# prime-slam/octreelib

Hardware: AMD Instinct MI355X
Metric: Mpoints/s insert+subdivide+RANSAC (higher is better)
Workload: dtype f64; 1 GPU; BASELINE config 3: Grid 1 m voxels, 10000000 planar points per GPU (scene 32x32x32 voxels), insert + subdivide(len>64) + map_leaf_points_cuda_ransac(H=1024, k=6, thr=0.01, poses_per_batch=10) incl. apply_mask; points_per_gpu=10000000, K=64, hypotheses=1024, leaves=575543

## Files before the change

octreelib_amd/csrc/ransac.hip:

```cpp
#include <algorithm>
#include <cstdlib>
#include <type_traits>

#include "forest.h"
#include "lookback.h"
#include "wave_utils.h"

namespace {

__device__ __forceinline__ double div_by_small_int(double c, int k) {
  const double kd = (double)k;
  const double zh = 1.0 / kd;
  const double zl = fma(-kd, zh, 1.0) / kd;
  const double a = fabs(c);
  if (!((int(a > 1e-290) | int(c == 0.0)) & int(a < 1e290))) return c / kd;
  return copysign(fma(c, zh, c * zl), c);
}

__device__ __forceinline__ bool coord_in_fast_range(double v) {
  const uint32_t hi = (uint32_t)__double2hiint(v), lo = (uint32_t)__double2loint(v);
  const uint32_t e = (hi >> 20) & 0x7FFu;
  return (e - (1023u - 30u)) <= 60u || (hi | lo) == 0u;
}

// ... 132 lines not shown
      if (i == 0) {
        xx = rx * rx;
        yy = ry * ry;
        zz = rz * rz;
      } else {
        xx += rx * rx;
        yy += ry * ry;
        zz += rz * rz;
      }
      xy += rx * ry;
      xz += rx * rz;
      yz += ry * rz;
    }
  }
  plane_from_moments(cx, cy, cz, xx, xy, xz, yy, yz, zz, plane, fast);
}

__device__ __forceinline__ double plane_distance(double a, double b, double c, double d, double x,
                                                 double y, double z) {
  return fabs(((a * x + b * y) + c * z) + d);
}

constexpr int rs_minwaves(int threads, int kt) { return threads == 64 && kt > 0 ? 5 : 4; }
constexpr int RS_BIG_PER_CU = 16;
constexpr int RS_BIG_THREADS = 256;
constexpr int RS_BIG_HPL = 1024 / RS_BIG_THREADS;
constexpr int RS_SMALL_THREADS = 128;
constexpr int RS_TINY_THREADS = 64;
constexpr int RS_PER_CU = 64, RS_SMALL_PER_CU = 128, RS_TINY_PER_CU = 256;
constexpr int RS_KMAX = 16;
constexpr int RS_STAGE1_SLACK = 2;
constexpr int RS_STAGE2_MIN = 6;
constexpr int RS_STAGE2_RING = 128;

struct __attribute__((aligned(32))) BlockDesc {
  uint32_t pstart;
  int32_t n;
  int64_t vstart;
  uint32_t pspill;
  uint32_t pad[3];
};

struct RansacOut {
  uint8_t* mask;
  float* plane;
  int32_t* count;
  int32_t* index;
};

__device__ __forceinline__ int sample_index_exact(double r, int n, int64_t vstart) {
  const double v = r * (double)n + (double)vstart;
  const int g = (int)((int64_t)(int)v - vstart);
  return g < n ? g : n;
}

__device__ __forceinline__ int sample_index_cached(double r, int n, bool* risky) {
  const double x = r * (double)n;
  const int g0 = (int)x;
  *risky = (x - (double)g0) > (1.0 - 0x1p-20);
  return g0 < n ? g0 : n;
}

__device__ __forceinline__ void plane_streamed(const double* __restrict__ hyp_row, int k, const BlockDesc& d,
                                               const double* __restrict__ xyz, float (&plane)[4]) {
  auto point = [&](int i) {
    const int g = sample_index_exact(hyp_row[i], d.n, d.vstart);
// ... 270 lines not shown
#ifdef RS_COUNTS
constexpr int RS_NSTAMPS = 24;
__device__ unsigned long long g_rs_stamps[RS_NSTAMPS];
#define RS_COUNT_INIT unsigned long long _rs_acc[RS_NSTAMPS] = {0, 0, 0, 0, 0, 0, 0, 0, 0, 0, 0, 0, 0, 0, 0, 0,  \
                                                                0, 0, 0, 0, 0, 0, 0, 0};                             \
                      const unsigned long long _rs_m0 = __builtin_amdgcn_s_memtime(),                      \
                                               _rs_r0 = __builtin_amdgcn_s_memrealtime()
#define RS_COUNT(k, v) _rs_acc[k] += (unsigned long long)(v)
#define RS_COUNT_FLUSH                                                                  \
  do {                                                                                  \
    if (threadIdx.x == 0) {                                                             \
      _rs_acc[0] = __builtin_amdgcn_s_memtime() - _rs_m0;                               \
      _rs_acc[1] = __builtin_amdgcn_s_memrealtime() - _rs_r0;                           \
      _rs_acc[10] += 1;                                                                 \
      for (int _k = 0; _k < RS_NSTAMPS; ++_k) atomicAdd(&g_rs_stamps[_k], _rs_acc[_k]); \
    }                                                                                   \
  } while (0)
#else
#define RS_COUNT_INIT do {} while (0)
#define RS_COUNT(k, v) do {} while (0)
#define RS_COUNT_FLUSH do {} while (0)
#endif

template <int THREADS, int HPL, int KT, bool FULLH, bool PT>
__global__ __launch_bounds__(THREADS, rs_minwaves(THREADS, KT)) void k_ransac(
    const double* __restrict__ xyz, const BlockDesc* __restrict__ sdesc,
    const uint32_t* __restrict__ lo_ptr, const uint32_t* __restrict__ hi_ptr, const double* __restrict__ hyp, int H,
    int k_rt, double thr, RansacOut out, const uint2* __restrict__ pos_tab, int no_prescreen) {
  static_assert(!PT || (KT > 0 && KT <= 6), "the position table packs up to six positions and their risk bits");
  static_assert(THREADS * HPL <= 1024, "hypothesis index in 10 bits");
  constexpr bool PRE = PT && KT >= 3 && HPL >= 2;
  constexpr int W = THREADS / 64;
  constexpr bool PARK = PRE && W == 1;
  constexpr int KS = KT > 0 ? KT : RS_KMAX;
  constexpr int GW = (KS + 3) / 4;
  constexpr int PRE_LIST = THREADS == 64 ? 512 : 256;
  constexpr bool OWN_LIST = PRE && W > 1;
  __shared__ uint16_t s_surv_all[OWN_LIST ? W : 1][OWN_LIST ? PRE_LIST : 1];
  uint16_t* const s_surv_own = s_surv_all[OWN_LIST ? (threadIdx.x >> 6) : 0];
  const int k = KT > 0 ? KT : k_rt;
  __shared__ double s_pts[3][3][THREADS];
  __shared__ uint32_t s_wbest[2][W];
  __shared__ float s_wplane[2][W][4];
  __shared__ f4 s_loc[3][THREADS];
  static_assert(!(PRE && W == 1) || PRE_LIST * sizeof(uint16_t) <= sizeof(s_loc[0]), "the survivor list fits an s_loc buffer");
  __shared__ float s_wext[3][W];
  __shared__ uint32_t s_wfast[3][W];
  const int lo = lo_ptr ? (int)*lo_ptr : 0;
  const int hi = (int)*hi_ptr;
  const int nbs = hi - lo;
  const int C = (nbs + (int)gridDim.x - 1) / (int)gridDim.x;
  int j = lo + (int)blockIdx.x * C;
  const int j_end = min(hi, j + C);
  if (j >= j_end) return;
  float ext_carry = 0.f;
  uint32_t fast_carry = 0;
  BlockDesc cur = sdesc[j];
  BlockDesc nxt = cur;
  if (j + 1 < j_end) nxt = sdesc[j + 1];
  {
    double px = 0.0, py = 0.0, pz = 0.0;
    if ((int)threadIdx.x <= cur.n) {
      const int64_t p = ((int)threadIdx.x < cur.n) ? (int64_t)cur.pstart + threadIdx.x : (int64_t)cur.pspill;
      px = xyz[3 * p];
      py = xyz[3 * p + 1];
      pz = xyz[3 * p + 2];
      s_pts[0][0][threadIdx.x] = px;
      s_pts[0][1][threadIdx.x] = py;
      s_pts[0][2][threadIdx.x] = pz;
    }
    stage_local<THREADS>(threadIdx.x, xyz[3 * (int64_t)cur.pstart], xyz[3 * (int64_t)cur.pstart + 1],
                         xyz[3 * (int64_t)cur.pstart + 2], cur, px, py, pz, s_loc[0], s_wext[0], s_wfast[0],
                         W == 1 ? &ext_carry : nullptr, W == 1 ? &fast_carry : nullptr);
  }
  __syncthreads();
  int buf = 0, par = 0;
  RS_COUNT_INIT;
  for (;;) {
    unsigned tx = threadIdx.x;
    asm volatile("" : "+v"(tx));
    const bool has_next = j + 1 < j_end;
    BlockDesc nxt2 = nxt;
    if (j + 2 < j_end) nxt2 = sdesc[j + 2];
    double rx = 0.0, ry = 0.0, rz = 0.0;
    auto pre_here = [&]() {
      unsigned t = tx;
      if constexpr (PARK) asm volatile("" : "+v"(t));
      return has_next && (int)t <= nxt.n;
    };
    const int nbuf = buf == 2 ? 0 : buf + 1;
    uint16_t* const s_surv = PARK ? (uint16_t*)&s_loc[nbuf][0] : s_surv_own;
    auto prefetch = [&]() {
      if (pre_here()) {
        const int64_t p = ((int)tx < nxt.n) ? (int64_t)nxt.pstart + tx : (int64_t)nxt.pspill;
        rx = xyz[3 * p];
        ry = xyz[3 * p + 1];
        rz = xyz[3 * p + 2];
      }
    };
    auto park = [&]() {
      if (pre_here()) {
        s_pts[nbuf][0][tx] = rx;
        s_pts[nbuf][1][tx] = ry;
        s_pts[nbuf][2][tx] = rz;
      }
    };
    double nox = 0.0, noy = 0.0, noz = 0.0;
    if constexpr (!PARK) {
      prefetch();
      if (has_next) {
        nox = xyz[3 * (int64_t)nxt.pstart];
        noy = xyz[3 * (int64_t)nxt.pstart + 1];
        noz = xyz[3 * (int64_t)nxt.pstart + 2];
      }
    }
    const int n = cur.n;
    const int be = (int)cur.pad[1];
    const double* __restrict__ lx = s_pts[buf][0];
    const double* __restrict__ ly = s_pts[buf][1];
    const double* __restrict__ lz = s_pts[buf][2];

    RS_COUNT(8, 1);
    RS_COUNT(11, n);
    float extent = W == 1 ? ext_carry : s_wext[buf][0];
#pragma unroll
    for (int w = 1; w < W; ++w) extent = fmaxf(extent, s_wext[buf][w]);
    uint32_t fastw = W == 1 ? fast_carry : s_wfast[buf][0];
#pragma unroll
    for (int w = 1; w < W; ++w) fastw &= s_wfast[buf][w];
    const bool blk_fast = __builtin_amdgcn_readfirstlane((int)fastw) != 0;
    const bool blk_sane = thr >= 0x1p-40 && thr <= 0x1p40 && extent < 0x1p60f;
    const bool fast_screen = blk_fast && thr >= 0x1p-40 && thr <= 0x1p40;
    const f4* __restrict__ loc = s_loc[buf];
    struct BlkConst {
      double ox, oy, oz;
      double delta_blk, dprime_thr, thr2;
      float nthr2;
      float delta_blk_f, thr2_f, dprime_thr_f;
    };
    auto blk_consts = [&]() {
      double th = thr;
      if constexpr (PARK) asm volatile("" : "+s"(th));
      BlkConst c;
      c.ox = lx[0]; c.oy = ly[0]; c.oz = lz[0];
      c.delta_blk = fma(0x1p-23 * 9.0, (double)extent,
                        0x1p-49 * (fabs(c.ox) + fabs(c.oy) + fabs(c.oz) + (double)extent + 1.0));
      c.dprime_thr = 0x1p-21 * (th * th);
      c.thr2 = th + th;
      c.nthr2 = -(float)(th * th);
      c.delta_blk_f = (float)c.delta_blk * 0x1.0002p0f;
      c.thr2_f = (float)(th + th) * 0x1.0002p0f;
      c.dprime_thr_f = (float)c.dprime_thr * 0x1.0002p0f;
      return c;
    };
    const BlkConst bc0 = blk_consts();
    auto consts_here = [&]() {
      if constexpr (PARK) return blk_consts();
      else return bc0;
    };
    const double ox = bc0.ox, oy = bc0.oy, oz = bc0.oz;

    uint32_t gpk[GW], rk = 0;
    float fa = 0.f, fb = 0.f, fc = 0.f, fd = 0.f, sto = 0.f, sdl = 0.f;
    int cnt = 0;
    auto load_pos = [&](const int t, const bool act) {
#pragma unroll
      for (int w = 0; w < GW; ++w) gpk[w] = 0;
      rk = 0;
      if constexpr (PT) {
        const uint2 e = pos_tab[(size_t)n * (size_t)H + (size_t)(act ? t : 0)];
        gpk[0] = e.x;
        if (GW > 1) gpk[GW - 1] = e.y & 0xFFFFu;
        rk = e.y >> 16;
      } else if (act) {
        const double* __restrict__ row = hyp + (int64_t)t * k;
#pragma unroll
        for (int i = 0; i < KS; ++i) {
          if (i < k) {
            bool risky;
            const int g = sample_index_cached(row[i], n, &risky);
            gpk[i >> 2] |= (uint32_t)g << (8 * (i & 3));
            rk |= (risky || g == n) ? (1u << i) : 0u;
          }
        }
      }
    };
    auto fit = [&](const int t, const bool act) {
      cnt = 0;
      fa = fb = fc = fd = sto = sdl = 0.f;
      if (FULLH || act) {
        const BlkConst bc = consts_here();
        const double ox = bc.ox, oy = bc.oy, oz = bc.oz, delta_blk = bc.delta_blk, dprime_thr = bc.dprime_thr;
        const float delta_blk_f = bc.delta_blk_f, thr2_f = bc.thr2_f, dprime_thr_f = bc.dprime_thr_f;
        double sx[KS], sy[KS], sz[KS];
        if (!__any(rk != 0u)) {
#pragma unroll
          for (int i = 0; i < KS; ++i) {
            sx[i] = sy[i] = sz[i] = 0.0;
            if (i < k) {
              const int g = (int)((gpk[i >> 2] >> (8 * (i & 3))) & 0xFFu);
              sx[i] = lx[g];
              sy[i] = ly[g];
              sz[i] = lz[g];
            }
          }
        } else {
#pragma unroll
          for (int i = 0; i < KS; ++i) {
            sx[i] = sy[i] = sz[i] = 0.0;
            if (i < k) {
              int g = (int)((gpk[i >> 2] >> (8 * (i & 3))) & 0xFFu);
              if (rk & (1u << i)) g = sample_index_exact(hyp[(int64_t)t * k + i], n, cur.vstart);
              sx[i] = lx[g];
              sy[i] = ly[g];
              sz[i] = lz[g];
            }
          }
        }
        float pf[4];
        plane_from_samples<KT, KS>(sx, sy, sz, k, pf, blk_fast);
        const double A = (double)pf[0], B = (double)pf[1], Cc = (double)pf[2], D = (double)pf[3];
        const double to = fma(A, ox, fma(B, oy, fma(Cc, oz, D)));
        fa = pf[0]; fb = pf[1]; fc = pf[2]; fd = pf[3];
        sto = (float)to;
        if (fast_screen) {
          const float dl = fma32(fabsf(sto), 0x1.0002p-21f, fma32(fabsf(pf[3]), 0x1.0002p-49f, delta_blk_f));
          sdl = fma32(dl, thr2_f + dl, dprime_thr_f) * 0x1.0002p0f;
        } else {
          const double delta = fma(0x1p-21, fabs(to), fma(0x1p-49, fabs(D), delta_blk));
          const double dprime = fma(delta, bc.thr2 + delta, dprime_thr) * 1.000001;
          const bool sane = blk_sane && (fabs(to) < 0x1p60);
          sdl = sane ? (float)dprime : __int_as_float(0x7f800000);
        }
      }
    };
    auto score = [&](const bool act) {
      float margin[1];
      int c1[1] = {0};
      RS_COUNT(14, 1);
      RS_COUNT(15, n);
      screen_group<1>(loc, n, &fa, &fb, &fc, &sto, consts_here().nthr2, c1, margin);
      cnt = c1[0];
      const bool redo = act && !(margin[0] > sdl);
      unsigned long long todo = __ballot(redo);
      RS_COUNT(13, __popcll(todo));
// ... 25 lines not shown
        }
      }
    };
    {
      const int t = (int)tx;
      const bool act = FULLH || t < H;
      load_pos(t, act);
      fit(t, act);
      if constexpr (PARK) prefetch();
      score(act);
      take(t, act);
    }
    if constexpr (HPL > 1) {
      int Lcur = (int)wave_max_u32((FULLH || (int)tx < H) ? (uint32_t)cnt : 0u);
      if (Lcur != n) {
        int S = 0;
        bool use_list = false;
        if constexpr (PRE) {
          PreConst pc;
          const bool elig = prescreen_constants(extent, ox, oy, oz, thr, pc) && blk_fast && !no_prescreen;
          if (elig) {
            RS_COUNT(4, 1);
            constexpr bool TWO = THREADS == 64;
            typedef uint32_t __attribute__((may_alias)) u32a;
            const int budget = n - Lcur;
            int m1 = n, qhead = 0, qtail = 0;
            bool two_stage = false;
            f4* ploc = nullptr;
            u32a *qlo = nullptr, *qhi = nullptr;
            if constexpr (TWO) {
              m1 = min(n, (budget + RS_STAGE1_SLACK + 3) & ~3);
              two_stage = n - m1 >= RS_STAGE2_MIN;
              if (two_stage) {
                const int third = buf == 0 ? 2 : buf - 1;
                ploc = s_loc[third];
                qlo = (u32a*)&s_pts[third][0][0];
                qhi = (u32a*)&s_pts[buf == 2 ? 0 : buf + 1][0][0];
                static_assert(3 * RS_STAGE2_RING * sizeof(uint32_t) <= sizeof(s_pts[0]), "three words per idle buffer");
                const unsigned long long wl = __ballot(cnt == Lcur);
                const int src = __ffsll((long long)wl) - 1;
                const float A = __uint_as_float(__builtin_amdgcn_readlane(__float_as_uint(fa), src));
                const float B = __uint_as_float(__builtin_amdgcn_readlane(__float_as_uint(fb), src));
                const float Cc = __uint_as_float(__builtin_amdgcn_readlane(__float_as_uint(fc), src));
                const float To = __uint_as_float(__builtin_amdgcn_readlane(__float_as_uint(sto), src));
                const bool mine = (int)tx < n;
                const f4 Lp = loc[mine ? tx : 0];
                const float sv = fma32(A, Lp.x, fma32(B, Lp.y, fma32(Cc, Lp.z, To)));
                const bool far = mine && !(fma32(sv, sv, consts_here().nthr2) < 0.f);
                const unsigned long long mf = __ballot(far), mn = __ballot(mine && !far);
                const unsigned long long mm = far ? mf : mn;
                const int pos = (far ? 0 : __popcll(mf)) +
                                (int)__builtin_amdgcn_mbcnt_hi((uint32_t)(mm >> 32), __builtin_amdgcn_mbcnt_lo((uint32_t)mm, 0u));
                if (mine) ploc[pos] = Lp;
                __builtin_amdgcn_fence(__ATOMIC_ACQ_REL, "wavefront");
              } else {
                RS_COUNT(19, 1);
              }
            }
            auto survive = [&](const bool sv, const uint32_t ub, const int t) {
              const unsigned long long mk = __ballot(sv);
              if (sv) {
                const int pos = S + (int)__builtin_amdgcn_mbcnt_hi((uint32_t)(mk >> 32), __builtin_amdgcn_mbcnt_lo((uint32_t)mk, 0u));
                if (pos < PRE_LIST) s_surv[pos] = (uint16_t)((ub << 10) | (uint32_t)t);
              }
              S += __popcll(mk);
            };
            auto stage2 = [&](const int nq) {
              __builtin_amdgcn_fence(__ATOMIC_ACQ_REL, "wavefront");
              const bool mine = (int)tx < nq;
              const int e = (qhead + (mine ? (int)tx : 0)) & (RS_STAGE2_RING - 1);
              const float a = __uint_as_float(qlo[e]), b = __uint_as_float(qlo[RS_STAGE2_RING + e]),
                          c = __uint_as_float(qlo[2 * RS_STAGE2_RING + e]), to = __uint_as_float(qhi[e]),
                          T2 = __uint_as_float(qhi[RS_STAGE2_RING + e]);
              const uint32_t w = qhi[2 * RS_STAGE2_RING + e];
              int c2[1] = {(int)(w >> 10)};
              screen_ub<1>(ploc + m1, n - m1, &a, &b, &c, &to, &T2, c2);
              RS_COUNT(17, 64 * (n - m1));
              RS_COUNT(21, 1);
              survive(mine && c2[0] > Lcur, (uint32_t)c2[0], (int)(w & 1023u));
              qhead += nq;
            };
            auto prescreen = [&](auto nh_tag, const int qb) {
              constexpr int NH = decltype(nh_tag)::value;
              uint2 pe[NH];
              auto hyp_a = [&](const int h) { return (int)tx + (qb + h) * THREADS; };
#pragma unroll
              for (int h = 0; h < NH; ++h)
                pe[h] = pos_tab[(size_t)n * (size_t)H + (size_t)((FULLH || hyp_a(h) < H) ? hyp_a(h) : 0)];
              float qa[NH], qb_[NH], qc[NH], qto[NH], qT2[NH];
              bool qok[NH];
              int qcnt[NH];
              uint32_t risk = 0;
#pragma unroll
              for (int h = 0; h < NH; ++h) {
                const uint32_t w0 = pe[h].x, w1 = pe[h].y;
                f4 P[KS];
#pragma unroll
                for (int i = 0; i < KS; ++i) P[i] = loc[((i < 4 ? w0 : w1) >> (8 * (i & 3))) & 0xFFu];
                const float inv_k = 1.0f / (float)KS;
                float cx = P[0].x, cy = P[0].y, cz = P[0].z;
#pragma unroll
                for (int i = 1; i < KS; ++i) {
                  cx += P[i].x;
                  cy += P[i].y;
                  cz += P[i].z;
                }
                cx *= inv_k;
                cy *= inv_k;
                cz *= inv_k;
                float xx, xy, xz, yy, yz, zz;
                {
                  const float ax = P[0].x - cx, ay = P[0].y - cy, az = P[0].z - cz;
                  xx = ax * ax; xy = ax * ay; xz = ax * az; yy = ay * ay; yz = ay * az; zz = az * az;
                }
#pragma unroll
                for (int i = 1; i < KS; ++i) {
                  const float ax = P[i].x - cx, ay = P[i].y - cy, az = P[i].z - cz;
                  xx = fma32(ax, ax, xx); xy = fma32(ax, ay, xy); xz = fma32(ax, az, xz);
                  yy = fma32(ay, ay, yy); yz = fma32(ay, az, yz); zz = fma32(az, az, zz);
                }
                const float dx = fma32(yy, zz, -(yz * yz)), dy = fma32(xx, zz, -(xz * xz)), dz = fma32(xx, yy, -(xy * xy));
                const float cA = fma32(xz, yz, -(xy * zz)), cB = fma32(xy, yz, -(xz * yy)), cC = fma32(xy, xz, -(yz * xx));
                const bool is_x = dx > dy && dx > dz;
                const bool is_y = !is_x && dy > dz;
                const float m1 = is_x ? dx : (is_y ? cA : cB);
                const float m2 = is_x ? cA : (is_y ? dy : cC);
                const float m3 = is_x ? cB : (is_y ? cC : dz);
                const float ss = fma32(m3, m3, fma32(m2, m2, m1 * m1));
                const float r = __builtin_amdgcn_rsqf(ss);
                const float a = m1 * r, b = m2 * r, c = m3 * r;
                qa[h] = a; qb_[h] = b; qc[h] = c;
                float to = -fma32(c, cz, fma32(b, cy, a * cx));
                asm volatile("" : "+v"(to));
                qto[h] = to;
                const float T = (xx + yy) + zz;
                const float mu4 = fma32(fma32(pc.qa, T, pc.qb), T, pc.qc);
                const float gap = __builtin_fmaxf(__builtin_fmaxf(dx, dy), dz) - __builtin_amdgcn_fmed3f(dx, dy, dz);
                qok[h] = (ss * r > mu4) && (gap > mu4);
                risk |= w1;
                const float thr_h = fma32(pc.e35, mu4 * r, pc.thrblk);
                qT2[h] = thr_h * thr_h;
                qcnt[h] = 0;
              }
              if (__any((risk >> 16) != 0u)) {
#pragma unroll
                for (int h = 0; h < NH; ++h) qok[h] = qok[h] && (pe[h].y >> 16) == 0u;
              }
              RS_COUNT(12, NH);
              RS_COUNT(22, 64 * NH * n);
              if constexpr (TWO) {
                if (two_stage) {
                  bool bad = false;
#pragma unroll
                  for (int h = 0; h < NH; ++h) bad = bad || !qok[h];
                  if (__any(bad)) {
#pragma unroll
                    for (int h = 0; h < NH; ++h) {
                      if (!qok[h]) {
                        qa[h] = qb_[h] = qc[h] = qto[h] = 0.f;
                        qT2[h] = 1.f;
                      }
                    }
                  }
                  screen_ub<NH>(ploc, m1, qa, qb_, qc, qto, qT2, qcnt);
                  RS_COUNT(16, 64 * NH * m1);
#pragma unroll
                  for (int h = 0; h < NH; ++h) {
                    const bool alive = qcnt[h] > m1 - budget && (FULLH || hyp_a(h) < H);
                    const unsigned long long mk = __ballot(alive);
                    if (alive) {
                      const int e = (qtail + (int)__builtin_amdgcn_mbcnt_hi((uint32_t)(mk >> 32), __builtin_amdgcn_mbcnt_lo((uint32_t)mk, 0u))) &
                                    (RS_STAGE2_RING - 1);
                      qlo[e] = __float_as_uint(qa[h]);
                      qlo[RS_STAGE2_RING + e] = __float_as_uint(qb_[h]);
                      qlo[2 * RS_STAGE2_RING + e] = __float_as_uint(qc[h]);
                      qhi[e] = __float_as_uint(qto[h]);
                      qhi[RS_STAGE2_RING + e] = __float_as_uint(qT2[h]);
                      qhi[2 * RS_STAGE2_RING + e] = ((uint32_t)qcnt[h] << 10) | (uint32_t)hyp_a(h);
                    }
// ... 62 lines not shown
      const int src = wl ? __ffsll((long long)wl) - 1 : 0;
      gbest = wbest;
      f0 = __uint_as_float(__builtin_amdgcn_readlane(__float_as_uint(wa), src));
      f1 = __uint_as_float(__builtin_amdgcn_readlane(__float_as_uint(wb), src));
      f2 = __uint_as_float(__builtin_amdgcn_readlane(__float_as_uint(wc), src));
      f3 = __uint_as_float(__builtin_amdgcn_readlane(__float_as_uint(wd), src));
      if (!wl) f0 = f1 = f2 = f3 = 0.f;
    } else if (best == wbest && best != 0) {
      const int w = tx >> 6;
      s_wbest[par][w] = best;
      s_wplane[par][w][0] = wa;
      s_wplane[par][w][1] = wb;
      s_wplane[par][w][2] = wc;
      s_wplane[par][w][3] = wd;
    } else if (wbest == 0 && (tx & 63) == 0) {
      s_wbest[par][tx >> 6] = 0;
    }
    if constexpr (PARK) {
      __builtin_amdgcn_fence(__ATOMIC_ACQ_REL, "wavefront");
      if (pre_here()) {
        rx = s_pts[nbuf][0][tx];
        ry = s_pts[nbuf][1][tx];
        rz = s_pts[nbuf][2][tx];
      }
      if (has_next) {
        nox = s_pts[nbuf][0][0];
        noy = s_pts[nbuf][1][0];
        noz = s_pts[nbuf][2][0];
      }
    } else {
      park();
    }
    if (has_next)
      stage_local<THREADS>(tx, nox, noy, noz, nxt, rx, ry, rz, s_loc[nbuf], s_wext[nbuf], s_wfast[nbuf],
                           W == 1 ? &ext_carry : nullptr, W == 1 ? &fast_carry : nullptr);
    __syncthreads();
    if constexpr (W > 1) {
      gbest = s_wbest[par][0];
      int gw = 0;
#pragma unroll
      for (int w = 1; w < W; ++w) {
        if (s_wbest[par][w] > gbest) {
          gbest = s_wbest[par][w];
          gw = w;
        }
      }
      f0 = s_wplane[par][gw][0]; f1 = s_wplane[par][gw][1]; f2 = s_wplane[par][gw][2]; f3 = s_wplane[par][gw][3];
    }
    if (tx == 0) {
      if (out.plane) {
        out.plane[4 * (int64_t)be + 0] = f0; out.plane[4 * (int64_t)be + 1] = f1;
        out.plane[4 * (int64_t)be + 2] = f2; out.plane[4 * (int64_t)be + 3] = f3;
      }
      if (out.count) out.count[be] = (int32_t)(gbest >> 10) - 1;
      if (out.index) out.index[be] = 1023 - (int)(gbest & 1023u);
    }
    if ((int)tx < n) {
      const double dist = plane_distance((double)f0, (double)f1, (double)f2, (double)f3,
                                         lx[tx], ly[tx], lz[tx]);
      out.mask[(int64_t)cur.pstart + tx] = (dist < thr) ? 1 : 0;
    }
    if (!has_next) break;
    cur = nxt;
    nxt = nxt2;
    j += 1;
    buf = nbuf;
    par ^= 1;
// ... 292 lines not shown
    uint32_t sp = d.n > 0 ? d.pstart + (uint32_t)d.n - 1u : d.pstart;
    if (phys[r + 1] >= 0) {
      sp = start[phys[r + 1]];
    } else if (!order) {
      const int64_t e = (int64_t)d.pstart + d.n;
      if (e < n_points) sp = (uint32_t)e;
    }
    d.pspill = sp;
    d.pad[0] = 0;
    d.pad[1] = (uint32_t)b;
    d.pad[2] = 0;
    desc[b] = d;
    if (d.n < k) {
      for (int i = 0; i < d.n; ++i) out.mask[(int64_t)d.pstart + i] = 0;
      if (out.plane) {
        out.plane[4 * b + 0] = 0.f; out.plane[4 * b + 1] = 0.f;
        out.plane[4 * b + 2] = 0.f; out.plane[4 * b + 3] = 0.f;
      }
      if (out.count) out.count[b] = 0;
      if (out.index) out.index[b] = -1;
    } else if (d.n > cap) {
      big_list[atomicAdd(&counters[RC_BIG], 1u)] = (uint32_t)b;
    } else {
      atomicAdd(&bins[d.n], 1u);
    }
    if (d.n >= k && (int64_t)d.n > max_block)
      __hip_atomic_store(&mirror[MIRROR_RS_VIOLATION], 1u, __ATOMIC_RELAXED, __HIP_MEMORY_SCOPE_SYSTEM);
  }
  __syncthreads();
  if (bins[threadIdx.x]) atomicAdd(&counters[RC_BINS + threadIdx.x], bins[threadIdx.x]);
}

__device__ __forceinline__ void pos_table_entry(const double* __restrict__ hyp, int H, int k,
                                                uint2* __restrict__ tab, int n, int t) {
  const double* __restrict__ row = hyp + (int64_t)t * k;
  uint32_t x = 0, y = 0;
  for (int i = 0; i < k; ++i) {
    bool risky;
    const uint32_t g = (uint32_t)sample_index_cached(row[i], n, &risky);
    if (i < 4) x |= g << (8 * i); else y |= g << (8 * (i - 4));
    y |= (risky || g == (uint32_t)n) ? (0x10000u << i) : 0u;
  }
  tab[(size_t)n * (size_t)H + t] = uint2{x, y};
}
__device__ __forceinline__ void pos_table_part(const double* __restrict__ hyp, int H, int k,
                                               const uint32_t* __restrict__ counters, uint2* __restrict__ tab,
                                               int n, int part) {
  const int t = part * 256 + (int)threadIdx.x;
  if (t >= H || n < k || counters[RC_BINS + n] == 0u) return;
  pos_table_entry(hyp, H, k, tab, n, t);
}

__global__ __launch_bounds__(256) void k_block_scatter(const BlockDesc* __restrict__ desc, int64_t nb,
                                                       int cap, int k,
                                                       uint32_t* __restrict__ counters,
                                                       BlockDesc* __restrict__ sdesc, unsigned n_scatter,
                                                       const double* __restrict__ hyp, int H,
                                                       uint2* __restrict__ tab, uint32_t* __restrict__ next_counters) {
  if (next_counters && blockIdx.x == gridDim.x - 1)
    for (int w = threadIdx.x; w < RC_WORDS; w += blockDim.x) next_counters[w] = 0;
  if (blockIdx.x >= n_scatter) {
    const unsigned parts = (unsigned)(H + 255) / 256u;
    const unsigned id = blockIdx.x - n_scatter;
    pos_table_part(hyp, H, k, counters, tab, (int)(id / parts), (int)(id % parts));
    return;
  }
  __shared__ uint32_t cnt[256];
  __shared__ uint32_t base[256];
  __shared__ uint32_t c[256];
  cnt[threadIdx.x] = 0;
  c[threadIdx.x] = counters[RC_BINS + threadIdx.x];
  __syncthreads();
  uint32_t first = 0;
  for (int m = 255; m > (int)threadIdx.x; --m) first += c[m];
  if (blockIdx.x == 0) {
    counters[RC_START + threadIdx.x] = first;
    if (threadIdx.x == 0) counters[RC_SORTED] = first + c[0];
  }
  constexpr int PER_THREAD = BS_PER_THREAD;
  const int64_t b0 = (int64_t)blockIdx.x * (256 * PER_THREAD);
  int nn[PER_THREAD];
  uint32_t rank[PER_THREAD];
#pragma unroll
  for (int r = 0; r < PER_THREAD; ++r) {
    const int64_t b = b0 + r * 256 + threadIdx.x;
    nn[r] = -1;
    rank[r] = 0;
    if (b < nb) {
      const int n = desc[b].n;
      if (n >= k && n <= cap) {
        nn[r] = n;
        rank[r] = atomicAdd(&cnt[n], 1u);
      }
    }
  }
  __syncthreads();
  if (cnt[threadIdx.x]) base[threadIdx.x] = first + atomicAdd(&counters[RC_FILL + threadIdx.x], cnt[threadIdx.x]);
  __syncthreads();
#pragma unroll
  for (int r = 0; r < PER_THREAD; ++r) {
    if (nn[r] >= 0) {
      const int64_t b = b0 + r * 256 + threadIdx.x;
      sdesc[base[nn[r]] + rank[r]] = desc[b];
    }
  }
}

constexpr int BPS_THREADS = 1024, BPS_MAX = BPS_THREADS * 8;
template <int BPS_PER_THREAD>
__global__ __launch_bounds__(BPS_THREADS) void k_block_prepare_small(
    const int32_t* __restrict__ order, const uint32_t* __restrict__ start, const int32_t* __restrict__ size,
    int64_t nb, int64_t n_points, int cap, int k, BlockDesc* __restrict__ desc, BlockDesc* __restrict__ sdesc,
    uint32_t* __restrict__ big_list, uint32_t* __restrict__ counters, RansacOut out, int64_t max_block,
    uint32_t* __restrict__ mirror, const double* __restrict__ hyp, int H, uint2* __restrict__ tab,
    uint32_t* __restrict__ next_counters) {
  if (blockIdx.x > 0) {
    const int parts = (H + BPS_THREADS - 1) / BPS_THREADS;
    const int id = (int)blockIdx.x - 1;
    const int n = k + id / parts, t = (id % parts) * BPS_THREADS + (int)threadIdx.x;
    if (t < H && n <= cap) pos_table_entry(hyp, H, k, tab, n, t);
    return;
  }
  __shared__ uint32_t bins[256];
  __shared__ uint32_t first[256];
  __shared__ uint32_t s_wave[BPS_THREADS / 64];
  if (next_counters)
    for (int w = threadIdx.x; w < RC_WORDS; w += BPS_THREADS) next_counters[w] = 0;
  if (threadIdx.x < 256) bins[threadIdx.x] = 0;
  const int lane = threadIdx.x & 63, wave = threadIdx.x >> 6;
  const int64_t b0 = (int64_t)threadIdx.x * BPS_PER_THREAD;
  int32_t phys[BPS_PER_THREAD + 1];
  int32_t nn[BPS_PER_THREAD];
#pragma unroll
  for (int r = 0; r <= BPS_PER_THREAD; ++r) {
    const int64_t b = b0 + r;
    phys[r] = b < nb ? (order ? order[b] : (int32_t)b) : -1;
  }
  uint32_t sum = 0;
#pragma unroll
  for (int r = 0; r < BPS_PER_THREAD; ++r) {
    nn[r] = phys[r] >= 0 ? size[phys[r]] : 0;
    sum += (uint32_t)nn[r];
  }
  uint32_t pst[BPS_PER_THREAD + 1];
#pragma unroll
  for (int r = 0; r <= BPS_PER_THREAD; ++r) pst[r] = phys[r] >= 0 ? start[phys[r]] : 0u;
  uint32_t inc = sum;
#pragma unroll
  for (int off = 1; off < 64; off <<= 1) {
    const uint32_t t = __shfl_up(inc, off);
    if (lane >= off) inc += t;
  }
  if (lane == 63) s_wave[wave] = inc;
// ... 69 lines not shown
    if (dd[r].n >= 0) sdesc[first[dd[r].n] + rank[r]] = dd[r];
}

}

int ransac_check_table(octl_ctx* ctx, const double* hyp, int32_t H, int32_t k) {
  const int64_t n = (int64_t)H * k;
  for (int64_t i = 0; i < n; ++i)
    if (!(hyp[i] >= 0.0 && hyp[i] < 1.0))
      return octl_set_error(ctx, OCTL_E_INVALID,
                            "hypothesis table entry %lld = %g is outside [0, 1): the table must hold "
                            "np.random.random draws (cuda_ransac.py:39-41)", (long long)i, hyp[i]);
  return OCTL_OK;
}

int ransac_launch(octl_ctx* ctx, const double* xyz_dev, int64_t n_points,
                  const uint32_t* blk_start, const int32_t* blk_size, const int32_t* order_dev,
                  int64_t nb, const double* hyp_dev, int32_t H, int32_t k, double thr,
                  uint8_t* mask_dev, float* plane_dev, int32_t* count_dev, int32_t* index_dev,
                  uint8_t* evaluated_dev, DevBuf& scratch, int64_t max_block) {
  (void)evaluated_dev;
  if (nb <= 0) return OCTL_OK;
  if (H < 1 || H > 1024) return octl_set_error(ctx, OCTL_E_INVALID, "H must be in [1, 1024]");
  if (k < 1) return octl_set_error(ctx, OCTL_E_INVALID, "initial_points_number must be positive");
  const bool any_k = k > RS_KMAX;
  if (nb >= ((int64_t)1 << 31)) return octl_set_error(ctx, OCTL_E_INVALID, "too many blocks");
  hipStream_t st = ctx->stream;
  const size_t off_d = (((size_t)nb + 8) * 4 + 31) & ~(size_t)31;
  const size_t off_s = off_d + (size_t)nb * sizeof(BlockDesc);
  const size_t off_b = off_s + (size_t)nb * sizeof(BlockDesc);
  const size_t off_c = (off_b + (size_t)nb * 4 + 31) & ~(size_t)31;
  const bool use_tab = !any_k && k >= 3 && k <= 6 && (H > 256 || k == 6);
  const size_t off_t = (off_c + RC_WORDS * 4 + 31) & ~(size_t)31;
  OCTL_TRY(devbuf_reserve(ctx, scratch, off_t + (use_tab ? (size_t)256 * (size_t)H * sizeof(uint2) : 0)));
  char* base = static_cast<char*>(scratch.p);
  uint32_t* tmp = scratch.as<uint32_t>();
  BlockDesc* desc = reinterpret_cast<BlockDesc*>(base + off_d);
  BlockDesc* sdesc = reinterpret_cast<BlockDesc*>(base + off_s);
  uint32_t* big_list = reinterpret_cast<uint32_t*>(base + off_b);
  uint32_t* counters = reinterpret_cast<uint32_t*>(base + off_c);
  const bool fused = !ctx->opt.no_fused_tables;
  uint32_t* next_counters = nullptr;
  if (fused) {
    if (!ctx->rs_counters.p || ctx->rs_counters_dirty) {
      OCTL_TRY(devbuf_reserve(ctx, ctx->rs_counters, (size_t)2 * RC_WORDS * 4));
      HIP_TRY(ctx, hipMemsetAsync(ctx->rs_counters.p, 0, (size_t)2 * RC_WORDS * 4, st));
      ctx->rs_parity = 0;
    }
    counters = ctx->rs_counters.as<uint32_t>() + (size_t)ctx->rs_parity * RC_WORDS;
    next_counters = ctx->rs_counters.as<uint32_t>() + (size_t)(ctx->rs_parity ^ 1) * RC_WORDS;
    ctx->rs_parity ^= 1;
    ctx->rs_counters_dirty = true;
  }
  uint2* pos_tab = use_tab ? reinterpret_cast<uint2*>(base + off_t) : nullptr;
  const int threads = (H <= 64) ? 64 : (H <= 256 ? 256 : RS_BIG_THREADS);
  RansacOut out{mask_dev, plane_dev, count_dev, index_dev};
  if (fused && nb <= BPS_MAX) {
    KTimer t(ctx, "ransac_prepare");
    const int cap = any_k ? 0 : threads - 1;
    const unsigned n_table = use_tab && cap >= k ? (unsigned)(cap - k + 1) * (unsigned)ceil_div(H, BPS_THREADS) : 0u;
    auto kp = nb <= 2 * BPS_THREADS ? k_block_prepare_small<2>
              : (nb <= 4 * BPS_THREADS ? k_block_prepare_small<4>
                                       : (nb <= 6 * BPS_THREADS ? k_block_prepare_small<6> : k_block_prepare_small<8>));
    OCTL_LAUNCH(kp, dim3(1 + n_table), dim3(BPS_THREADS), 0, st, order_dev, blk_start, blk_size, nb,
                       n_points, cap, (int)k, desc, sdesc, big_list, counters, out, max_block,
                       static_cast<uint32_t*>(ctx->small_host), hyp_dev, (int)H, pos_tab, next_counters);
    HIP_TRY(ctx, hipGetLastError());
    ctx->rs_counters_dirty = false;
  } else {
    KTimer t(ctx, "ransac_prepare");
    if (fused) {
      const unsigned g = (unsigned)ceil_div(nb, 256 * BP_PER_THREAD);
      uint64_t* status = nullptr;
      uint32_t epoch = 0;
      OCTL_TRY(octl_scan_status_acquire(ctx, g, &status, &epoch));
      OCTL_LAUNCH(k_block_prepare, dim3(g), dim3(256), 0, st, order_dev, blk_start, blk_size, nb, n_points,
                         any_k ? 0 : threads - 1, (int)k, desc, big_list, counters, out, status, epoch, max_block,
                         static_cast<uint32_t*>(ctx->small_host));
      HIP_TRY(ctx, hipGetLastError());
    } else {
      const unsigned g = (unsigned)ceil_div(nb, 256);
      OCTL_LAUNCH(k_block_sizes_in_order, dim3(g), dim3(256), 0, st, order_dev, blk_size, nb, tmp, counters);
      HIP_TRY(ctx, hipGetLastError());
      OCTL_TRY(octl_exclusive_scan_u32(ctx, tmp, tmp, nb, nullptr));
      OCTL_LAUNCH(k_block_desc, dim3((unsigned)ceil_div(nb, 256 * BD_PER_THREAD)), dim3(256), 0, st, order_dev,
                         blk_start, blk_size,
                         (const uint32_t*)tmp, nb, n_points, any_k ? 0 : threads - 1, (int)k, desc, big_list,
                         counters, out);
      HIP_TRY(ctx, hipGetLastError());
    }
    const unsigned n_scatter = (unsigned)ceil_div(nb, 256 * BS_PER_THREAD);
    const unsigned n_table = use_tab ? 256u * (unsigned)ceil_div(H, 256) : 0u;
    OCTL_LAUNCH(k_block_scatter, dim3(n_scatter + n_table), dim3(256), 0, st,
                       (const BlockDesc*)desc, nb, any_k ? 0 : threads - 1, (int)k, counters, sdesc, n_scatter, hyp_dev,
                       (int)H, pos_tab, next_counters);
    HIP_TRY(ctx, hipGetLastError());
    ctx->rs_counters_dirty = false;
  }
  const int cus = octl_ctx_cus(ctx);
  KTimer t(ctx, "ransac");
  hipStream_t side = st;
  bool on_side = false;
  int waves_per_block = (int)ctx->opt.ransac_waves;
  if (waves_per_block == 0 && !any_k && H > 256) {
    const int64_t slots = (int64_t)cus * 16;
    if (nb * 2 <= slots) waves_per_block = 4;
    else if (nb <= 6 * slots) waves_per_block = 2;
  }
  const bool need_small = max_block >= RS_TINY_THREADS, need_mid = max_block >= RS_SMALL_THREADS,
             need_big = any_k || max_block >= threads;
  const bool side_work = waves_per_block == 4 ? need_big
                         : (waves_per_block == 2 ? (need_mid || need_big) : (need_small || need_mid || need_big));
  if (!any_k && H > 256 && side_work && octl_ctx_side_stream(ctx) &&
      hipEventRecord(ctx->self_gate, st) == hipSuccess &&
      hipStreamWaitEvent(ctx->self_stream, ctx->self_gate, 0) == hipSuccess) {
    side = ctx->self_stream;
    on_side = true;
  }
  const int no_prescreen = ctx->opt.no_ransac_prescreen ? 1 : 0;
#define OCTL_RANSAC_RANGE(THREADS, HPL, KT, PER_CU, LO, HI, PT, ST)                              \
  do {                                                                                           \
    const unsigned g = (unsigned)std::min<int64_t>(nb, (int64_t)cus * (PER_CU));                 \
    if (H == (THREADS) * (HPL))                                                                  \
      OCTL_LAUNCH((k_ransac<THREADS, HPL, KT, true, PT>), dim3(g), dim3(THREADS), 0, ST,         \
                         xyz_dev, (const BlockDesc*)sdesc, (const uint32_t*)(LO), (const uint32_t*)(HI), \
                         hyp_dev, H, k, thr, out, (const uint2*)pos_tab, no_prescreen);           \
    else                                                                                         \
      OCTL_LAUNCH((k_ransac<THREADS, HPL, KT, false, PT>), dim3(g), dim3(THREADS), 0, ST,        \
                         xyz_dev, (const BlockDesc*)sdesc, (const uint32_t*)(LO), (const uint32_t*)(HI), \
                         hyp_dev, H, k, thr, out, (const uint2*)pos_tab, no_prescreen);           \
  } while (0)
#define OCTL_RANSAC_LAUNCH(THREADS, HPL, KT, PER_CU, PT) \
  OCTL_RANSAC_RANGE(THREADS, HPL, KT, PER_CU, nullptr, counters + RC_SORTED, PT, st)
#define OCTL_RANSAC_SPLIT(KT)                                                                                    \
  do {                                                                                                           \
    if (waves_per_block == 4) {                                                                                  \
      OCTL_RANSAC_RANGE(RS_BIG_THREADS, RS_BIG_HPL, KT, RS_PER_CU, nullptr, counters + RC_SORTED, true, st);     \
    } else if (waves_per_block == 2) {                                                                           \
      if (need_mid)                                                                                              \
        OCTL_RANSAC_RANGE(RS_BIG_THREADS, RS_BIG_HPL, KT, RS_PER_CU, nullptr,                                    \
                          counters + RC_START + RS_SMALL_THREADS - 1, true, side);                               \
// ... 148 lines not shown
```

Measured before the change: 3855 Mpoints/s.

## Use pre-scaled byte-offset position table and fixed LDS buffers in single-wave RANSAC

```diff
diff --git a/octreelib_amd/csrc/ransac.hip b/octreelib_amd/csrc/ransac.hip
--- a/octreelib_amd/csrc/ransac.hip
+++ b/octreelib_amd/csrc/ransac.hip
@@ -188,6 +188,9 @@
 constexpr int RS_STAGE1_SLACK = 2;
 constexpr int RS_STAGE2_MIN = 6;
 constexpr int RS_STAGE2_RING = 128;
+constexpr int PS_FIRST = 256;
+constexpr int PS_BITS = 10;
+constexpr uint32_t PS_FLAG = 1u << 30;
 
 struct __attribute__((aligned(32))) BlockDesc {
   uint32_t pstart;
@@ -524,8 +527,9 @@
   constexpr bool PRE = PT && KT >= 3 && HPL >= 2;
   constexpr int W = THREADS / 64;
   constexpr bool PARK = PRE && W == 1;
+  constexpr bool FIXED = PARK;
   constexpr int KS = KT > 0 ? KT : RS_KMAX;
-  constexpr int GW = (KS + 3) / 4;
+  constexpr int GW = FIXED ? 2 : (KS + 3) / 4;
   constexpr int PRE_LIST = THREADS == 64 ? 512 : 256;
   constexpr bool OWN_LIST = PRE && W > 1;
   __shared__ uint16_t s_surv_all[OWN_LIST ? W : 1][OWN_LIST ? PRE_LIST : 1];
@@ -580,8 +584,12 @@
       if constexpr (PARK) asm volatile("" : "+v"(t));
       return has_next && (int)t <= nxt.n;
     };
-    const int nbuf = buf == 2 ? 0 : buf + 1;
-    uint16_t* const s_surv = PARK ? (uint16_t*)&s_loc[nbuf][0] : s_surv_own;
+    const int cbuf = FIXED ? par : buf;
+    const int nbuf = FIXED ? (par ^ 1) : (buf == 2 ? 0 : buf + 1);
+    const int tbuf = FIXED ? 2 : (buf == 0 ? 2 : buf - 1);
+    constexpr int LOC_FIXED = 0, PLOC_FIXED = 1, SURV_FIXED = 2;
+    f4* const loc_next = FIXED ? s_loc[LOC_FIXED] : s_loc[nbuf];
+    uint16_t* const s_surv = PARK ? (uint16_t*)&s_loc[SURV_FIXED][0] : s_surv_own;
     auto prefetch = [&]() {
       if (pre_here()) {
         const int64_t p = ((int)tx < nxt.n) ? (int64_t)nxt.pstart + tx : (int64_t)nxt.pspill;
@@ -608,9 +616,9 @@
     }
     const int n = cur.n;
     const int be = (int)cur.pad[1];
-    const double* __restrict__ lx = s_pts[buf][0];
-    const double* __restrict__ ly = s_pts[buf][1];
-    const double* __restrict__ lz = s_pts[buf][2];
+    const double* __restrict__ lx = s_pts[cbuf][0];
+    const double* __restrict__ ly = s_pts[cbuf][1];
+    const double* __restrict__ lz = s_pts[cbuf][2];
 
     RS_COUNT(8, 1);
     RS_COUNT(11, n);
@@ -623,7 +631,7 @@
     const bool blk_fast = __builtin_amdgcn_readfirstlane((int)fastw) != 0;
     const bool blk_sane = thr >= 0x1p-40 && thr <= 0x1p40 && extent < 0x1p60f;
     const bool fast_screen = blk_fast && thr >= 0x1p-40 && thr <= 0x1p40;
-    const f4* __restrict__ loc = s_loc[buf];
+    std::conditional_t<FIXED, const f4*, const f4* __restrict__> loc = FIXED ? s_loc[LOC_FIXED] : s_loc[buf];
     struct BlkConst {
       double ox, oy, oz;
       double delta_blk, dprime_thr, thr2;
@@ -659,7 +667,12 @@
 #pragma unroll
       for (int w = 0; w < GW; ++w) gpk[w] = 0;
       rk = 0;
-      if constexpr (PT) {
+      if constexpr (FIXED) {
+        const uint2 e = pos_tab[((size_t)PS_FIRST + (size_t)n) * (size_t)H + (size_t)(act ? t : 0)];
+        gpk[0] = e.x;
+        gpk[1] = e.y;
+        rk = e.y & PS_FLAG;
+      } else if constexpr (PT) {
         const uint2 e = pos_tab[(size_t)n * (size_t)H + (size_t)(act ? t : 0)];
         gpk[0] = e.x;
         if (GW > 1) gpk[GW - 1] = e.y & 0xFFFFu;
@@ -685,15 +698,24 @@
         const double ox = bc.ox, oy = bc.oy, oz = bc.oz, delta_blk = bc.delta_blk, dprime_thr = bc.dprime_thr;
         const float delta_blk_f = bc.delta_blk_f, thr2_f = bc.thr2_f, dprime_thr_f = bc.dprime_thr_f;
         double sx[KS], sy[KS], sz[KS];
+        auto byte_off = [&](const int i) { return (gpk[i / 3] >> (PS_BITS * (i % 3) + 1)) & 0x1FFu; };
+        auto at = [](const double* base, const uint32_t off) { return *(const double*)((const char*)base + off); };
         if (!__any(rk != 0u)) {
 #pragma unroll
           for (int i = 0; i < KS; ++i) {
             sx[i] = sy[i] = sz[i] = 0.0;
             if (i < k) {
-              const int g = (int)((gpk[i >> 2] >> (8 * (i & 3))) & 0xFFu);
-              sx[i] = lx[g];
-              sy[i] = ly[g];
-              sz[i] = lz[g];
+              if constexpr (FIXED) {
+                const uint32_t off = byte_off(i);
+                sx[i] = at(lx, off);
+                sy[i] = at(ly, off);
+                sz[i] = at(lz, off);
+              } else {
+                const int g = (int)((gpk[i >> 2] >> (8 * (i & 3))) & 0xFFu);
+                sx[i] = lx[g];
+                sy[i] = ly[g];
+                sz[i] = lz[g];
+              }
             }
           }
         } else {
@@ -701,8 +723,18 @@
           for (int i = 0; i < KS; ++i) {
             sx[i] = sy[i] = sz[i] = 0.0;
             if (i < k) {
-              int g = (int)((gpk[i >> 2] >> (8 * (i & 3))) & 0xFFu);
-              if (rk & (1u << i)) g = sample_index_exact(hyp[(int64_t)t * k + i], n, cur.vstart);
+              int g;
+              if constexpr (FIXED) {
+                g = (int)(byte_off(i) >> 3);
+                if (rk) {
+                  bool risky;
+                  const int g0 = sample_index_cached(hyp[(int64_t)t * k + i], n, &risky);
+                  if (risky || g0 == n) g = sample_index_exact(hyp[(int64_t)t * k + i], n, cur.vstart);
+                }
+              } else {
+                g = (int)((gpk[i >> 2] >> (8 * (i & 3))) & 0xFFu);
+                if (rk & (1u << i)) g = sample_index_exact(hyp[(int64_t)t * k + i], n, cur.vstart);
+              }
               sx[i] = lx[g];
               sy[i] = ly[g];
               sz[i] = lz[g];
@@ -794,10 +826,9 @@
               m1 = min(n, (budget + RS_STAGE1_SLACK + 3) & ~3);
               two_stage = n - m1 >= RS_STAGE2_MIN;
               if (two_stage) {
-                const int third = buf == 0 ? 2 : buf - 1;
-                ploc = s_loc[third];
-                qlo = (u32a*)&s_pts[third][0][0];
-                qhi = (u32a*)&s_pts[buf == 2 ? 0 : buf + 1][0][0];
+                ploc = FIXED ? s_loc[PLOC_FIXED] : s_loc[tbuf];
+                qlo = (u32a*)&s_pts[tbuf][0][0];
+                qhi = (u32a*)&s_pts[nbuf][0][0];
                 static_assert(3 * RS_STAGE2_RING * sizeof(uint32_t) <= sizeof(s_pts[0]), "three words per idle buffer");
                 const unsigned long long wl = __ballot(cnt == Lcur);
                 const int src = __ffsll((long long)wl) - 1;
@@ -848,17 +879,24 @@
               auto hyp_a = [&](const int h) { return (int)tx + (qb + h) * THREADS; };
 #pragma unroll
               for (int h = 0; h < NH; ++h)
-                pe[h] = pos_tab[(size_t)n * (size_t)H + (size_t)((FULLH || hyp_a(h) < H) ? hyp_a(h) : 0)];
+                pe[h] = pos_tab[((size_t)(FIXED ? PS_FIRST : 0) + (size_t)n) * (size_t)H +
+                                (size_t)((FULLH || hyp_a(h) < H) ? hyp_a(h) : 0)];
               float qa[NH], qb_[NH], qc[NH], qto[NH], qT2[NH];
               bool qok[NH];
               int qcnt[NH];
+              auto flagged = [](const uint32_t w1) { return FIXED ? (w1 & PS_FLAG) : (w1 >> 16); };
               uint32_t risk = 0;
 #pragma unroll
               for (int h = 0; h < NH; ++h) {
                 const uint32_t w0 = pe[h].x, w1 = pe[h].y;
                 f4 P[KS];
 #pragma unroll
-                for (int i = 0; i < KS; ++i) P[i] = loc[((i < 4 ? w0 : w1) >> (8 * (i & 3))) & 0xFFu];
+                for (int i = 0; i < KS; ++i) {
+                  if constexpr (FIXED)
+                    P[i] = *(const f4*)((const char*)loc + (((i < 3 ? w0 : w1) >> (PS_BITS * (i % 3))) & ((1u << PS_BITS) - 1u)));
+                  else
+                    P[i] = loc[((i < 4 ? w0 : w1) >> (8 * (i & 3))) & 0xFFu];
+                }
                 const float inv_k = 1.0f / (float)KS;
                 float cx = P[0].x, cy = P[0].y, cz = P[0].z;
 #pragma unroll
@@ -904,9 +942,9 @@
                 qT2[h] = thr_h * thr_h;
                 qcnt[h] = 0;
               }
-              if (__any((risk >> 16) != 0u)) {
-#pragma unroll
-                for (int h = 0; h < NH; ++h) qok[h] = qok[h] && (pe[h].y >> 16) == 0u;
+              if (__any(flagged(risk) != 0u)) {
+#pragma unroll
+                for (int h = 0; h < NH; ++h) qok[h] = qok[h] && flagged(pe[h].y) == 0u;
               }
               RS_COUNT(12, NH);
               RS_COUNT(22, 64 * NH * n);
@@ -1035,7 +1073,7 @@
       park();
     }
     if (has_next)
-      stage_local<THREADS>(tx, nox, noy, noz, nxt, rx, ry, rz, s_loc[nbuf], s_wext[nbuf], s_wfast[nbuf],
+      stage_local<THREADS>(tx, nox, noy, noz, nxt, rx, ry, rz, loc_next, s_wext[nbuf], s_wfast[nbuf],
                            W == 1 ? &ext_carry : nullptr, W == 1 ? &fast_carry : nullptr);
     __syncthreads();
     if constexpr (W > 1) {
@@ -1394,23 +1432,25 @@
 }
 
 __device__ __forceinline__ void pos_table_entry(const double* __restrict__ hyp, int H, int k,
-                                                uint2* __restrict__ tab, int n, int t) {
+                                                uint2* __restrict__ tab, int n, int t, int ps) {
   const double* __restrict__ row = hyp + (int64_t)t * k;
-  uint32_t x = 0, y = 0;
+  uint32_t x = 0, y = 0, a = 0, b = 0;
   for (int i = 0; i < k; ++i) {
     bool risky;
     const uint32_t g = (uint32_t)sample_index_cached(row[i], n, &risky);
     if (i < 4) x |= g << (8 * i); else y |= g << (8 * (i - 4));
     y |= (risky || g == (uint32_t)n) ? (0x10000u << i) : 0u;
+    if (i < 3) a |= (g << 4) << (PS_BITS * i); else b |= (g << 4) << (PS_BITS * (i - 3));
   }
   tab[(size_t)n * (size_t)H + t] = uint2{x, y};
+  if (ps && n < RS_TINY_THREADS) tab[((size_t)PS_FIRST + (size_t)n) * (size_t)H + t] = uint2{a, (y >> 16) ? (b | PS_FLAG) : b};
 }
 __device__ __forceinline__ void pos_table_part(const double* __restrict__ hyp, int H, int k,
                                                const uint32_t* __restrict__ counters, uint2* __restrict__ tab,
-                                               int n, int part) {
+                                               int n, int part, int ps) {
   const int t = part * 256 + (int)threadIdx.x;
   if (t >= H || n < k || counters[RC_BINS + n] == 0u) return;
-  pos_table_entry(hyp, H, k, tab, n, t);
+  pos_table_entry(hyp, H, k, tab, n, t, ps);
 }
 
 __global__ __launch_bounds__(256) void k_block_scatter(const BlockDesc* __restrict__ desc, int64_t nb,
@@ -1418,13 +1458,14 @@
                                                        uint32_t* __restrict__ counters,
                                                        BlockDesc* __restrict__ sdesc, unsigned n_scatter,
                                                        const double* __restrict__ hyp, int H,
-                                                       uint2* __restrict__ tab, uint32_t* __restrict__ next_counters) {
+                                                       uint2* __restrict__ tab, uint32_t* __restrict__ next_counters,
+                                                       int ps) {
   if (next_counters && blockIdx.x == gridDim.x - 1)
     for (int w = threadIdx.x; w < RC_WORDS; w += blockDim.x) next_counters[w] = 0;
   if (blockIdx.x >= n_scatter) {
     const unsigned parts = (unsigned)(H + 255) / 256u;
     const unsigned id = blockIdx.x - n_scatter;
-    pos_table_part(hyp, H, k, counters, tab, (int)(id / parts), (int)(id % parts));
+    pos_table_part(hyp, H, k, counters, tab, (int)(id / parts), (int)(id % parts), ps);
     return;
   }
   __shared__ uint32_t cnt[256];
@@ -1475,12 +1516,12 @@
     int64_t nb, int64_t n_points, int cap, int k, BlockDesc* __restrict__ desc, BlockDesc* __restrict__ sdesc,
     uint32_t* __restrict__ big_list, uint32_t* __restrict__ counters, RansacOut out, int64_t max_block,
     uint32_t* __restrict__ mirror, const double* __restrict__ hyp, int H, uint2* __restrict__ tab,
-    uint32_t* __restrict__ next_counters) {
+    uint32_t* __restrict__ next_counters, int ps) {
   if (blockIdx.x > 0) {
     const int parts = (H + BPS_THREADS - 1) / BPS_THREADS;
     const int id = (int)blockIdx.x - 1;
     const int n = k + id / parts, t = (id % parts) * BPS_THREADS + (int)threadIdx.x;
-    if (t < H && n <= cap) pos_table_entry(hyp, H, k, tab, n, t);
+    if (t < H && n <= cap) pos_table_entry(hyp, H, k, tab, n, t, ps);
     return;
   }
   __shared__ uint32_t bins[256];
@@ -1616,7 +1657,8 @@
   const size_t off_c = (off_b + (size_t)nb * 4 + 31) & ~(size_t)31;
   const bool use_tab = !any_k && k >= 3 && k <= 6 && (H > 256 || k == 6);
   const size_t off_t = (off_c + RC_WORDS * 4 + 31) & ~(size_t)31;
-  OCTL_TRY(devbuf_reserve(ctx, scratch, off_t + (use_tab ? (size_t)256 * (size_t)H * sizeof(uint2) : 0)));
+  OCTL_TRY(devbuf_reserve(ctx, scratch,
+                          off_t + (use_tab ? (size_t)(PS_FIRST + RS_TINY_THREADS) * (size_t)H * sizeof(uint2) : 0)));
   char* base = static_cast<char*>(scratch.p);
   uint32_t* tmp = scratch.as<uint32_t>();
   BlockDesc* desc = reinterpret_cast<BlockDesc*>(base + off_d);
@@ -1637,6 +1679,14 @@
     ctx->rs_counters_dirty = true;
   }
   uint2* pos_tab = use_tab ? reinterpret_cast<uint2*>(base + off_t) : nullptr;
+  const int cus = octl_ctx_cus(ctx);
+  int waves_per_block = (int)ctx->opt.ransac_waves;
+  if (waves_per_block == 0 && !any_k && H > 256) {
+    const int64_t slots = (int64_t)cus * 16;
+    if (nb * 2 <= slots) waves_per_block = 4;
+    else if (nb <= 6 * slots) waves_per_block = 2;
+  }
+  const int ps_tab = (use_tab && H > 256 && waves_per_block != 2 && waves_per_block != 4) ? 1 : 0;
   const int threads = (H <= 64) ? 64 : (H <= 256 ? 256 : RS_BIG_THREADS);
   RansacOut out{mask_dev, plane_dev, count_dev, index_dev};
   if (fused && nb <= BPS_MAX) {
@@ -1648,7 +1698,7 @@
                                        : (nb <= 6 * BPS_THREADS ? k_block_prepare_small<6> : k_block_prepare_small<8>));
     OCTL_LAUNCH(kp, dim3(1 + n_table), dim3(BPS_THREADS), 0, st, order_dev, blk_start, blk_size, nb,
                        n_points, cap, (int)k, desc, sdesc, big_list, counters, out, max_block,
-                       static_cast<uint32_t*>(ctx->small_host), hyp_dev, (int)H, pos_tab, next_counters);
+                       static_cast<uint32_t*>(ctx->small_host), hyp_dev, (int)H, pos_tab, next_counters, ps_tab);
     HIP_TRY(ctx, hipGetLastError());
     ctx->rs_counters_dirty = false;
   } else {
@@ -1677,20 +1727,13 @@
     const unsigned n_table = use_tab ? 256u * (unsigned)ceil_div(H, 256) : 0u;
     OCTL_LAUNCH(k_block_scatter, dim3(n_scatter + n_table), dim3(256), 0, st,
                        (const BlockDesc*)desc, nb, any_k ? 0 : threads - 1, (int)k, counters, sdesc, n_scatter, hyp_dev,
-                       (int)H, pos_tab, next_counters);
+                       (int)H, pos_tab, next_counters, ps_tab);
     HIP_TRY(ctx, hipGetLastError());
     ctx->rs_counters_dirty = false;
   }
-  const int cus = octl_ctx_cus(ctx);
   KTimer t(ctx, "ransac");
   hipStream_t side = st;
   bool on_side = false;
-  int waves_per_block = (int)ctx->opt.ransac_waves;
-  if (waves_per_block == 0 && !any_k && H > 256) {
-    const int64_t slots = (int64_t)cus * 16;
-    if (nb * 2 <= slots) waves_per_block = 4;
-    else if (nb <= 6 * slots) waves_per_block = 2;
-  }
   const bool need_small = max_block >= RS_TINY_THREADS, need_mid = max_block >= RS_SMALL_THREADS,
              need_big = any_k || max_block >= threads;
   const bool side_work = waves_per_block == 4 ? need_big
```

New measurement: 3894 Mpoints/s (median of 6 runs). 1.01x the previous value.
